# r-mafi/ClaraGenomicsAnalysis

Hardware: AMD Instinct MI355X
Metric: POA windows/sec (consensus) (higher is better)
Workload: dtype int16

## Files before the change

### claragenomicsanalysis_amd/csrc/poa_common.hpp

```cpp
#pragma once

#include <cstddef>
#include <cstdint>

namespace gwamd
{
namespace poa
{

constexpr int kMaxEdges      = 50;
constexpr int kMaxAlignments = 50;
constexpr int kBandPad       = 8;
constexpr int kWave          = 64;
constexpr int kCellsPerLane  = 8;
constexpr int kChunk         = kWave * kCellsPerLane;
constexpr int kAdRing        = 128;
constexpr int kAdSpillDist   = kAdRing - kWave + 1;
constexpr int band_ring_rows(int cpl) { return cpl >= 16 ? 8 : 16; }
constexpr int band_tile_rows(int cpl) { return cpl >= 10 ? 32 : 64; }
constexpr int kReadGuard     = 64;
constexpr int kAdMaxWaves    = 4;
constexpr int kColShift      = 7;

enum Status : uint8_t
{
    kSuccess               = 0,
    kExceededMaxPoas       = 1,
    kExceededMaxSeqSize    = 2,
    kExceededMaxSeqsPerPoa = 3,
    kNodeCountExceeded     = 4,
    kEdgeCountExceeded     = 5,
    kSeqLenExceededNodes   = 6,
    kLoopCountExceeded     = 7,
    kOutputTypeUnavailable = 8,
    kGenericError          = 9,
};

struct WindowDesc
{
    int32_t first_seq;
    int32_t num_seqs;
};

struct Dims
{
    int32_t max_nodes;
    int32_t max_seqs;
    int32_t max_seq_len;
    int32_t max_consensus;
    int32_t score_stride;
    int32_t score_rows;
    int32_t aln_cap;
    int32_t band_width;
    int32_t want_consensus;
    int32_t spoa_accurate;
    int32_t lds_kernel;
    int32_t lds_bytes;
    int32_t lds_ring_off;
    int32_t lds_ring_rows;
    int32_t lds_sh_off;
    int32_t lds_rec_off;
    int32_t lds_xl_off;
    int32_t lds_xl_cap;
    int32_t lds_cpl;
    int32_t lds_waves;
    int32_t code_stride;
    int64_t aux_stride;
    int32_t aux_carry_off;
    int32_t lds_work_bytes;
    int32_t aux_reca_off;
    int32_t aux_recb_off;
    int32_t aux_col0_off;
    int32_t aux_flag_off;
    int32_t aux_xl_off;
    int32_t aux_xl_cap;
    int32_t aux_bx_off;
    int32_t aux_recc_off;
    int32_t aux_rece_off;
    int32_t band_ad;
    int32_t tb_rank;
    int32_t diag;
};

constexpr int kTbRanked     = 1;
constexpr int kTbStrips     = 2;
constexpr int kTbStrip32    = 4;
constexpr int kTbDefault    = kTbRanked | kTbStrips;
constexpr int kTbAboveShift = 3;
constexpr int kTbAboveMask  = 7;

constexpr int kDiagTopsortRing  = 1;
constexpr int kDiagFwdV1        = 2;
constexpr int kDiagTopsortFifo  = 4;
constexpr int kDiagRaconV1      = 8;
constexpr int kDiagConsensusHbm = 16;
constexpr int kDiagAddWave0     = 32;
constexpr int kDiagAddSerial    = 64;
constexpr int kDiagOrderKahn    = 128;
constexpr int kDiagSinkCap2     = 256;
constexpr int kDiagConsLdsShift = 16;

struct LdsShape
{
    int cpl, waves;
    bool wide;
};
constexpr LdsShape kLdsShapes[] = {{8, 1, true},   {8, 2, true},   {8, 4, true},   {8, 8, true},  {16, 8, true},
                                   {8, 1, false},  {16, 1, false}, {24, 1, false}, {32, 1, false}, {8, 2, false},
                                   {8, 3, false},  {8, 4, false},  {16, 4, false}, {4, 4, false}};
constexpr int kNumLdsShapes = int(sizeof(kLdsShapes) / sizeof(kLdsShapes[0]));

struct KernelRef
{
    const void* fn;
    int threads;
    size_t dynamic_lds;
};

constexpr int64_t lds_read_bytes(int64_t max_seq_len) { return (max_seq_len + 48 + 15) & ~int64_t(15); }

constexpr int kAddShBytes = 64;
constexpr int64_t lds_add_ms(int64_t max_seq_len) { return (max_seq_len + 16) & ~int64_t(15); }
constexpr int64_t lds_add_wave0_bytes(int64_t max_seq_len, int64_t max_nodes)
{
    return 5 * lds_add_ms(max_seq_len) + 2 * (max_nodes + max_seq_len);
}
constexpr int64_t lds_add_hit_off(int64_t max_seq_len, int64_t max_nodes)
{
    return (lds_add_wave0_bytes(max_seq_len, max_nodes) + 15) & ~int64_t(15);
}
constexpr int64_t lds_add_bytes(int64_t max_seq_len, int64_t max_nodes)
{
    return lds_add_hit_off(max_seq_len, max_nodes) + 2 * lds_add_ms(max_seq_len) + kAddShBytes;
}
constexpr bool lds_add_fits(int64_t max_seq_len, int64_t max_nodes, int64_t ring_bytes)
{
    return max_seq_len > 0 && max_nodes > 0 && max_nodes + max_seq_len < 65535 &&
           lds_add_bytes(max_seq_len, max_nodes) <= ring_bytes;
}

constexpr int kTbRankBytes = 7 * 144 + 128 * 4;

constexpr int kShProg    = 16;
constexpr int kShEnd     = 32;
constexpr int kShBnd     = 64;
constexpr int kShChan    = 128;
constexpr int kChanRows  = 64;
constexpr int kMaxWaves  = 4;
constexpr int kShBytes(int waves) { return kShChan + (waves - 1) * kChanRows * 4; }
constexpr int kShEndW   = 32;
constexpr int kShProgW  = 64;
constexpr int kShBndW   = 128;
constexpr int kShChanW  = 384;
constexpr int kMaxRingW = 8;
constexpr int kShBytesW(int waves) { return kShChanW + (waves - 1) * kChanRows * 8; }

constexpr int kTileRows = 128;
constexpr int kTileCols = 128;
constexpr int kTileXlMin = 512;

struct Buffers
{
    const uint8_t* seqs;
    const int8_t* wts;
    const int32_t* seq_len;
    const int64_t* seq_off;
    const WindowDesc* windows;
    const int32_t* order;
    int32_t num_windows;
    int32_t* head;
    int32_t num_slots;
    uint8_t* base;
    uint16_t* in_cnt;
    uint16_t* out_cnt;
    uint16_t* aln_cnt;
    uint16_t* node_cov;
    uint16_t* in_w;
    void* in_e;
    void* out_e;
    void* aln;
    void* sorted;
    void* pos;
    void* ag;
    void* ar;
    void* scores;
    uint8_t* codes;
    int32_t* cscore;
    void* cpred;
    uint16_t* edge_cov;
    uint16_t* edge_cov_cnt;
    void* seq_begin;
    uint8_t* cons;
    uint16_t* cov;
    int32_t* cons_len;
    uint8_t* status;
    uint8_t* msa_status;
    uint8_t* msa;
    int32_t* msa_len;
    int32_t* final_nodes;
    int64_t* cells;
    int64_t* phase;
    int32_t* order_stats;
};

enum OrderStat
{
    kOsSpliced = 0,
    kOsSortSeqAdd,
    kOsSortCheck,
    kOsSortNoOld,
    kOsSortSinkCap,
    kOsSortEmptyRead,
    kOsSortLast,
    kOsTieSorts,
    kOsTieQuick,
    kOsSortAfterTie,
    kOrderStats
};


enum Phase
{
    kPhBackbone = 0,
    kPhForward,
    kPhTraceback,
    kPhAdd,
    kPhTopsort,
    kPhOutput,
// ... 13 lines not shown
```

### claragenomicsanalysis_amd/csrc/poa_fwd2.hpp

```cpp
#pragma once

__device__ __forceinline__ bool fwd2_ok(const Scores sc)
{
    const int s_eq = sc.match - sc.gap, s_ne = sc.mismatch - sc.gap;
    return s_eq >= 0 && s_eq <= 255 && s_ne >= 0 && s_ne <= 255;
}

__device__ __forceinline__ int wave_incl_max_b(int v)
{
    v = max(v, __builtin_amdgcn_update_dpp(INT_MIN, v, 0x111, 0xf, 0xf, false));
    v = max(v, __builtin_amdgcn_update_dpp(INT_MIN, v, 0x112, 0xf, 0xf, false));
    v = max(v, __builtin_amdgcn_update_dpp(INT_MIN, v, 0x114, 0xf, 0xf, false));
    v = max(v, __builtin_amdgcn_update_dpp(INT_MIN, v, 0x118, 0xf, 0xf, false));
    v = max(v, __builtin_amdgcn_update_dpp(INT_MIN, v, 0x142, 0xa, 0xf, false));
    v = max(v, __builtin_amdgcn_update_dpp(INT_MIN, v, 0x143, 0xc, 0xf, false));
    return v;
}

typedef u32x4 fwd_u32x4;
typedef u32x2 fwd_u32x2;

template <int NR>
__device__ __forceinline__ void load_row_glb(const GWAMD_GLB int16_t* p, uint32_t (&P)[NR], uint32_t& prev)
{
    static_assert(NR % 4 == 0 || NR == 2, "4 or a multiple of 8 cells per lane");
    if constexpr (NR % 4 == 0)
    {
#pragma unroll
        for (int q = 0; q < NR / 4; q++)
        {
            const fwd_u32x4 v = *reinterpret_cast<const GWAMD_GLB fwd_u32x4*>(p + 1 + 8 * q);
            P[4 * q] = v.x, P[4 * q + 1] = v.y, P[4 * q + 2] = v.z, P[4 * q + 3] = v.w;
        }
    }
    else
    {
        const fwd_u32x2 v = *reinterpret_cast<const GWAMD_GLB fwd_u32x2*>(p + 1);
        P[0] = v.x, P[1] = v.y;
    }
    prev = uint32_t(uint16_t(p[0]));
}

template <int NR>
__device__ __forceinline__ void load_row_lds(const GWAMD_LDS int16_t* p, uint32_t (&P)[NR], uint32_t& prev)
{
    static_assert(NR % 4 == 0 || NR == 2, "4 or a multiple of 8 cells per lane");
    if constexpr (NR % 4 == 0)
    {
#pragma unroll
        for (int q = 0; q < NR / 4; q++)
        {
            const fwd_u32x4 v = *reinterpret_cast<const GWAMD_LDS fwd_u32x4*>(p + 1 + 8 * q);
            P[4 * q] = v.x, P[4 * q + 1] = v.y, P[4 * q + 2] = v.z, P[4 * q + 3] = v.w;
        }
    }
    else
    {
        const fwd_u32x2 v = *reinterpret_cast<const GWAMD_LDS fwd_u32x2*>(p + 1);
        P[0] = v.x, P[1] = v.y;
    }
    prev = uint32_t(uint16_t(p[0]));
}

template <int CPL, int NW, bool FIRST, bool FEED, typename SizeT>
__device__ __forceinline__ void fwd2_rows(WinGraph<SizeT> g, const RowProg& P, int V, const uint8_t* read_f, int L,
                                          int16_t* ring_f, int ring_stride, int16_t* spill_f, int stride,
                                          uint8_t* codes_f, int code_stride, const Scores sc,
                                          GWAMD_LDS uint8_t* shb, int16_t* carry_f, int lane, int wave, int cb,
                                          bool to_hbm, bool from_hbm, bool owner, int xl_cap, int& best_row,
                                          int& best_val)
{
    g = as_global(g);
    GWAMD_LDS int16_t* ring          = lds_of(ring_f);
    const GWAMD_LDS uint8_t* read    = lds_of(read_f);
    const GWAMD_LDS uint32_t* prec   = lds_of(P.rec);
    const GWAMD_LDS uint16_t* pxl    = lds_of(P.xl);
    GWAMD_GLB int16_t* spill         = (GWAMD_GLB int16_t*)(spill_f);
    GWAMD_GLB uint8_t* codes         = (GWAMD_GLB uint8_t*)(codes_f);
    GWAMD_GLB int16_t* carry_hbm     = (GWAMD_GLB int16_t*)(carry_f);
    constexpr int NR    = CPL / 2;
    const int gap       = sc.gap;
    const int s_eq      = sc.match - gap;
    const int s_ne      = sc.mismatch - gap;
    const uint32_t gap2 = pk_bcast(gap);
    const uint32_t one2 = opaque_u32(0x00010001u);
    const uint32_t two2 = opaque_u32(0x00020002u);
    const int mask      = uniform(P.ring_mask);
    GWAMD_LDS int16_t* bnd               = (GWAMD_LDS int16_t*)(shb + kShBnd) + wave * (mask + 1);
    GWAMD_LDS uint32_t* chan             = (GWAMD_LDS uint32_t*)(shb + kShChan);
    volatile GWAMD_LDS uint32_t* chan_in  = chan + (wave - 1) * kChanRows;
    volatile GWAMD_LDS uint32_t* chan_out = chan + wave * kChanRows;
    volatile GWAMD_LDS int* prog_v        = (GWAMD_LDS int*)(shb + kShProg);
    const int jb     = cb + lane * CPL;
    const bool active = jb < L;
    const int ja     = active ? jb : 0;
    const int own_lane = ((L > 0 ? L - 1 : 0) % (kWave * CPL)) / CPL;
    const int own_c    = (L > 0 ? L - 1 : 0) % CPL;
    const int xl_last = xl_cap;

    uint32_t T[CPL];
#pragma unroll
    for (int c = 0; c < CPL; c++)
    {
        const int ch = int(read[ja + c]);
        T[c] = uint32_t(ch == 'A' ? s_eq : s_ne) | (uint32_t(ch == 'C' ? s_eq : s_ne) << 8) |
               (uint32_t(ch == 'T' ? s_eq : s_ne) << 16) | (uint32_t(ch == 'G' ? s_eq : s_ne) << 24);
    }
    uint32_t Eprev[NR];
#pragma unroll
    for (int i = 0; i < NR; i++)
        Eprev[i] = 0;
    int cin_prev = 0;
    int hbm_c    = 0;
    uint32_t rec_c = uint32_t(uniform(int(prec[1])));
    uint32_t rec_n = uint32_t(uniform(int(prec[min(2, V)])));
    auto xls_at = [&](int i) { return int(pxl[i]); };
    int pv_c = xls_at(min(int(rec_c >> 16), xl_last) + lane);
    GWAMD_GLB uint8_t* crow = codes + code_stride;
    GWAMD_GLB int16_t* srow = spill + stride;
    for (int r = 1; r <= V; r++, crow += code_stride, srow += stride)
    {
        const uint32_t rec = rec_c;
        const uint32_t rec_nn = prec[min(r + 2, V)];
        const int pv_n = xls_at(min(int(rec_n >> 16), xl_last) + lane);
        const int np       = int((rec >> 8) & 63);
        const bool spill_r = (rec >> 15) & 1;
        GWAMD_LDS int16_t* row = ring + (r & mask) * ring_stride;
        uint32_t sig[NR];
        {
            const uint32_t bsel = 0x0c040c00u + ((rec >> 1) & 3u) * 0x00010001u;
#pragma unroll
            for (int i = 0; i < NR; i++)
                sig[i] = __builtin_amdgcn_perm(T[2 * i + 1], T[2 * i], bsel);
        }
        int cin = 0;
        auto finish = [&](auto multi_tag, const uint32_t(&dg)[NR], const uint32_t(&vt)[NR],
                          const uint32_t(&kd)[NR], const uint32_t(&kv)[NR], int c0v,
                          int c0kv) __attribute__((always_inline)) {
            constexpr bool kMulti = decltype(multi_tag)::value;
            uint32_t E[NR];
#pragma unroll
            for (int i = 0; i < NR; i++)
            {
                const uint32_t s = pk_max_lo_into_hi(pk_max(dg[i], vt[i]));
                E[i]             = i == 0 ? s : pk_max_hi_carry(s, E[i - 1]);
            }
            const int m    = active ? int(int16_t(E[NR - 1] >> 16)) : kNeg;
            const int incl = wave_incl_max_b(m);
            const int excl = __builtin_amdgcn_update_dpp(kNeg, incl, 0x138, 0xf, 0xf, false);
            const int wtot = __builtin_amdgcn_readlane(incl, kWave - 1);
            if (FIRST)
            {
                cin = c0v + gap;
                if (lane == 0)
                {
                    row[kColShift]  = int16_t(cin);
                    crow[kColShift] = uint8_t(1 | (c0kv << 2));
                    if (spill_r)
                        srow[kColShift] = int16_t(cin);
                }
            }
            else
            {
                if (from_hbm)
                {
                    if (((r - 1) & (kWave - 1)) == 0)
                    {
                        const int x = r + lane;
                        uint32_t hc = x <= V ? uint32_t(int(carry_hbm[x])) : 0u;
                        settle_vm1(hc);
                        hbm_c = int(hc);
                    }
                    cin = int(int16_t(__builtin_amdgcn_readlane(hbm_c, (r - 1) & (kWave - 1))));
                }
                else
                {
                    uint32_t w = uint32_t(uniform(int(chan_in[r & (kChanRows - 1)])));
                    while ((w >> 16) != (uint32_t(r) & 0xffffu))
                    {
                        __builtin_amdgcn_s_sleep(1);
                        w = uint32_t(uniform(int(chan_in[r & (kChanRows - 1)])));
                    }
                    cin = int(int16_t(w & 0xffffu));
                    if ((r & 7) == 0 && lane == 0)
                        prog_v[wave] = r;
                }
                if (lane == 0)
                {
                    bnd[r & mask] = int16_t(cin);
                    if (spill_r)
                        srow[cb + kColShift] = int16_t(cin);
                }
            }
            if (FEED)
            {
                if ((r & 31) == 0 && r >= kChanRows)
                {
                    while (uniform(prog_v[wave + 1]) < r - 32)
                        __builtin_amdgcn_s_sleep(1);
                }
                if (lane == 0)
                    chan_out[r & (kChanRows - 1)] = (uint32_t(r) << 16) | uint32_t(uint16_t(max(cin, wtot)));
            }
            if (to_hbm && lane == 0)
                carry_hbm[r] = int16_t(max(cin, wtot));
            const uint32_t b2v = pk_bcast(max(excl, cin));
#pragma unroll
            for (int i = 0; i < NR; i++)
                E[i] = pk_max(E[i], b2v);
            if (active)
            {
                uint32_t code[NR];
#pragma unroll
                for (int i = 0; i < NR; i++)
                {
                    if constexpr (kMulti)
                    {
                        const uint32_t a   = pk_min_u(pk_sub(E[i], dg[i]), one2);
                        const uint32_t bb  = pk_min_u(pk_sub(E[i], vt[i]), one2);
                        const uint32_t cvh = pk_mad(bb, pk_sub(two2, kv[i]), kv[i]);
                        code[i]            = pk_mad(a, pk_sub(cvh, kd[i]), kd[i]);
                    }
                    else
                    {
                        const uint32_t a = pk_min_u(pk_sub(E[i], dg[i]), one2);
                        code[i]          = pk_add(a, pk_min_u(pk_sub(E[i], vt[i]), a));
                    }
                }
                if constexpr (NR % 4 == 0)
                {
#pragma unroll
                    for (int q = 0; q < NR / 4; q++)
                    {
                        const fwd_u32x4 ev = {E[4 * q], E[4 * q + 1], E[4 * q + 2], E[4 * q + 3]};
                        *reinterpret_cast<GWAMD_LDS fwd_u32x4*>(row + jb + kColShift + 1 + 8 * q) = ev;
                        if (spill_r)
                            *reinterpret_cast<GWAMD_GLB fwd_u32x4*>(srow + jb + kColShift + 1 + 8 * q) = ev;
                        const uint32_t w0 = __builtin_amdgcn_perm(code[4 * q + 1], code[4 * q], 0x06040200u);
                        const uint32_t w1 = __builtin_amdgcn_perm(code[4 * q + 3], code[4 * q + 2], 0x06040200u);
                        __builtin_nontemporal_store(uint64_t(w0) | (uint64_t(w1) << 32),
                                                    reinterpret_cast<GWAMD_GLB uint64_t*>(crow + jb + kColShift + 1 + 8 * q));
                    }
                }
                else
                {
                    const fwd_u32x2 ev = {E[0], E[1]};
                    *reinterpret_cast<GWAMD_LDS fwd_u32x2*>(row + jb + kColShift + 1) = ev;
                    if (spill_r)
                        *reinterpret_cast<GWAMD_GLB fwd_u32x2*>(srow + jb + kColShift + 1) = ev;
                    __builtin_nontemporal_store(__builtin_amdgcn_perm(code[1], code[0], 0x06040200u),
                                                reinterpret_cast<GWAMD_GLB uint32_t*>(crow + jb + kColShift + 1));
                }
            }
            if ((rec & (1u << 14)) && owner)
            {
                int endv = cin;
#pragma unroll
                for (int i = 0; i < NR; i++)
                {
                    if (2 * i == own_c)
                        endv = int(int16_t(E[i] & 0xffff));
                    if (2 * i + 1 == own_c)
                        endv = int(int16_t(E[i] >> 16));
                }
                const int v = L == 0 ? cin : __builtin_amdgcn_readlane(endv, own_lane);
                if (best_val < v)
                    best_val = v, best_row = r;
            }
#pragma unroll
            for (int i = 0; i < NR; i++)
                Eprev[i] = E[i];
        };
        if (!(rec & 0x80u) && np == 1)
        {
            const int d = int(rec >> 16);
            uint32_t prev;
            if (d == 1)
                prev = uint32_t(__builtin_amdgcn_update_dpp(int(uint32_t(uint16_t(cin_prev))),
                                                            int(Eprev[NR - 1] >> 16), 0x138, 0xf, 0xf, false));
            else
            {
                const int ps = (r - d) & mask;
                load_row_lds<NR>(ring + ps * ring_stride + ja + kColShift, Eprev, prev);
                if (!FIRST)
                {
                    const uint32_t bv = uint32_t(uint16_t(bnd[ps]));
                    prev              = lane == 0 ? bv : prev;
                }
            }
            const int c0v = FIRST ? int(int16_t(__builtin_amdgcn_readfirstlane(prev))) : 0;
            uint32_t dg[NR], vt[NR];
            diag_src<NR>(Eprev, prev, dg);
#pragma unroll
            for (int i = 0; i < NR; i++)
            {
                dg[i] = pk_add(dg[i], sig[i]);
                vt[i] = pk_add(Eprev[i], gap2);
            }
            finish(std::false_type{}, dg, vt, dg, vt, c0v, 0);
        }
        else
        {
            auto rows_general = [&](auto slow_tag, int pv, int n) __attribute__((always_inline)) {
                constexpr bool kSlow = decltype(slow_tag)::value;
                auto load_pred = [&](int p, uint32_t(&Q)[NR], uint32_t& qprev) __attribute__((always_inline)) {
                    if (p == r - 1)
                    {
#pragma unroll
                        for (int i = 0; i < NR; i++)
                            Q[i] = Eprev[i];
                        qprev = uint32_t(__builtin_amdgcn_update_dpp(int(uint32_t(uint16_t(cin_prev))),
                                                                     int(Eprev[NR - 1] >> 16), 0x138, 0xf, 0xf,
                                                                     false));
                        return;
                    }
                    if constexpr (kSlow)
                    {
                        if (p == 0)
                        {
#pragma unroll
                            for (int i = 0; i < NR; i++)
                                Q[i] = 0;
                            qprev = 0;
                            return;
                        }
                        if (r - p > mask)
                        {
                            load_row_glb<NR>(spill + size_t(p) * stride + ja + kColShift, Q, qprev);
                            settle_vm<NR>(Q, qprev);
                            return;
                        }
                    }
                    load_row_lds<NR>(ring + (p & mask) * ring_stride + ja + kColShift, Q, qprev);
                    if (!FIRST)
                    {
                        const uint32_t bv = uint32_t(uint16_t(bnd[p & mask]));
                        qprev             = lane == 0 ? bv : qprev;
                    }
                };
                uint32_t dg[NR], vt[NR];
                int c0v = 0, c0kv = 0;
                {
                    uint32_t Pv[NR], prev;
                    load_pred(__builtin_amdgcn_readfirstlane(pv), Pv, prev);
                    if (FIRST)
                        c0v = int(int16_t(__builtin_amdgcn_readfirstlane(prev)));
                    diag_src<NR>(Pv, prev, dg);
#pragma unroll
                    for (int i = 0; i < NR; i++)
                    {
                        dg[i] = pk_add(dg[i], sig[i]);
                        vt[i] = pk_add(Pv[i], gap2);
                    }
                }
                if (n > 1)
                {
                    uint32_t kd[NR], kv[NR];
#pragma unroll
                    for (int i = 0; i < NR; i++)
                    {
                        kd[i] = 0;
                        kv[i] = one2;
                    }
                    for (int k = 1; k < n; k++)
                    {
                        uint32_t Q[NR], qprev, dq[NR];
                        load_pred(__builtin_amdgcn_readlane(pv, k), Q, qprev);
                        if (FIRST)
                        {
                            const int pe = int(int16_t(__builtin_amdgcn_readfirstlane(qprev)));
                            c0kv         = pe > c0v ? k : c0kv;
                            c0v          = max(c0v, pe);
                        }
                        diag_src<NR>(Q, qprev, dq);
                        const uint32_t kk4 = pk_bcast(4 * k);
                        const uint32_t kk1 = pk_bcast(4 * k + 1);
#pragma unroll
                        for (int i = 0; i < NR; i++)
                        {
                            const uint32_t d  = pk_add(dq[i], sig[i]);
                            const uint32_t nd = pk_max(dg[i], d);
                            kd[i] = pk_mad(pk_min_u(pk_sub(nd, dg[i]), one2), pk_sub(kk4, kd[i]), kd[i]);
                            dg[i] = nd;
                            const uint32_t v  = pk_add(Q[i], gap2);
                            const uint32_t nv = pk_max(vt[i], v);
                            kv[i] = pk_mad(pk_min_u(pk_sub(nv, vt[i]), one2), pk_sub(kk1, kv[i]), kv[i]);
                            vt[i] = nv;
                        }
                    }
                    finish(std::true_type{}, dg, vt, kd, kv, c0v, c0kv);
                }
                else
                    finish(std::false_type{}, dg, vt, dg, vt, c0v, 0);
            };
            if (!(rec & 0x80u))
                rows_general(std::false_type{}, pv_c, np);
            else
            {
                int n  = np;
                int pv = 0;
                if (np == int(kRecEscape))
                    pv = row_preds<SizeT>(P, g, r, rec, lane, n);
                else
                {
                    if (np >= 2)
                        pv = lane < np ? int(pxl[(rec >> 16) + lane]) : 0;
                    else if (np == 1)
                        pv = r - int(rec >> 16);
                    if (np == 0)
                        n = 1;
                }
                const uint32_t ub = uint32_t(row_base<SizeT>(g, rec, r));
                if (!((ub & 0xc0u) == 0x40u && ((0x10008aull >> (ub & 0x3fu)) & 1u)))
                {
                    const GWAMD_LDS uint32_t* rw = reinterpret_cast<const GWAMD_LDS uint32_t*>(read + ja);
#pragma unroll
                    for (int i = 0; i < NR; i++)
                    {
                        const uint32_t wv = rw[i / 2] >> ((i & 1) * 16);
                        const int ch0 = int(wv & 0xff), ch1 = int((wv >> 8) & 0xff);
                        sig[i]        = uint32_t(uint16_t(ch0 == int(ub) ? s_eq : s_ne)) |
                                 (uint32_t(uint16_t(ch1 == int(ub) ? s_eq : s_ne)) << 16);
                    }
                }
                rows_general(std::true_type{}, pv, uniform(n));
            }
        }
        cin_prev = cin;
        rec_c    = rec_n;
        rec_n    = uint32_t(uniform(int(rec_nn)));
        pv_c     = pv_n;
    }
}

template <int CPL, int NW, typename SizeT>
__device__ int nw_forward_lds_v2(WinGraph<SizeT> g, const RowProg& P, int V, const uint8_t* read, int L,
                                 int16_t* ring, int ring_stride, int16_t* spill, int stride, uint8_t* codes,
                                 int code_stride, const Scores sc, GWAMD_LDS uint8_t* shb, int16_t* carry_hbm,
                                 int tid, int xl_cap)
{
    constexpr int kSpan = kWave * CPL;
    const int lane      = tid & (kWave - 1);
    const int wave      = uniform(tid / kWave);
    V                   = uniform(V);
    L                   = uniform(L);
    const int jl        = L > 0 ? L - 1 : 0;
    const int own_span  = jl / kSpan;
    const int nspan     = max(1, (L + kSpan - 1) / kSpan);
    const int nsweep    = (nspan + NW - 1) / NW;
    int best_row        = 0;
    int best_val        = INT_MIN;
    for (int sweep = 0; sweep < nsweep; sweep++)
    {
        if (sweep > 0)
        {
            __syncthreads();
            for (int t = tid; t < (kShChan - kShProg) / 4 + (NW - 1) * kChanRows; t += kWave * NW)
                reinterpret_cast<GWAMD_LDS int*>(shb + kShProg)[t] = 0;
            __syncthreads();
        }
        const int span      = sweep * NW + wave;
        const int cb        = span * kSpan;
        const bool first    = span == 0;
        const bool wact     = cb < L || first;
        const bool feed     = wave + 1 < NW && cb + kSpan < L;
        const bool to_hbm   = wave == NW - 1 && cb + kSpan < L;
        const bool from_hbm = wave == 0 && sweep > 0;
        const bool owner    = span == own_span;
        if (!wact || V < 1)
            continue;
        if (first)
        {
            if (feed)
                fwd2_rows<CPL, NW, true, true>(g, P, V, read, L, ring, ring_stride, spill, stride, codes,
                                               code_stride, sc, shb, carry_hbm, lane, wave, cb, to_hbm, from_hbm,
                                               owner, xl_cap, best_row, best_val);
            else
                fwd2_rows<CPL, NW, true, false>(g, P, V, read, L, ring, ring_stride, spill, stride, codes,
                                                code_stride, sc, shb, carry_hbm, lane, wave, cb, to_hbm,
                                                from_hbm, owner, xl_cap, best_row, best_val);
        }
        else if (feed)
            fwd2_rows<CPL, NW, false, true>(g, P, V, read, L, ring, ring_stride, spill, stride, codes, code_stride,
                                            sc, shb, carry_hbm, lane, wave, cb, to_hbm, from_hbm, owner, xl_cap,
                                            best_row, best_val);
        else
            fwd2_rows<CPL, NW, false, false>(g, P, V, read, L, ring, ring_stride, spill, stride, codes,
                                             code_stride, sc, shb, carry_hbm, lane, wave, cb, to_hbm, from_hbm,
                                             owner, xl_cap, best_row, best_val);
    }
    if (nsweep > 1 || NW > 1)
    {
        GWAMD_LDS int* endp = (GWAMD_LDS int*)(shb + kShEnd);
        if (wave == own_span % NW && lane == 0)
            *endp = best_row;
        __syncthreads();
        best_row = uniform(*endp);
    }
    return best_row;
}
```

### claragenomicsanalysis_amd/csrc/poa_kernels.hip

```cpp
#include <hip/hip_runtime.h>

#include <climits>
#include <cstdint>
#include <type_traits>
#include <utility>

#include "poa_wave.hpp"
#include "poa_order.hpp"
#include "poa_rowprog.hpp"

namespace gwamd
{
namespace poa
{

template <typename ScoreT, typename SizeT, bool BANDED, bool MSA>
__global__ void __launch_bounds__(kWave) poa_window_kernel(Buffers b, Dims d, Scores sc)
{
    extern __shared__ __align__(16) uint8_t lds_read[];
    __shared__ int sh_alen;
    __shared__ int sh_status;
    __shared__ int sh_len;

    const int w = b.order ? b.order[blockIdx.x] : int(blockIdx.x);
// ... 154 lines not shown
    return __builtin_bit_cast(uint32_t, __builtin_elementwise_min(__builtin_bit_cast(pk_u16x2, a),
                                                                  __builtin_bit_cast(pk_u16x2, b)));
}
__device__ __forceinline__ uint32_t pk_mad(uint32_t a, uint32_t b, uint32_t c)
{
    return __builtin_bit_cast(uint32_t, __builtin_bit_cast(pk_u16x2, a) * __builtin_bit_cast(pk_u16x2, b) +
                                            __builtin_bit_cast(pk_u16x2, c));
}
__device__ __forceinline__ uint32_t opaque_u32(uint32_t v)
{
    asm volatile("" : "+v"(v));
    return v;
}
__device__ __forceinline__ uint32_t pk_bcast(int v) { return (uint32_t(uint16_t(v)) * 0x10001u); }
__device__ __forceinline__ uint32_t pk_max_lo_into_hi(uint32_t a)
{
    const pk_s16x2 v = __builtin_bit_cast(pk_s16x2, a);
    return __builtin_bit_cast(uint32_t, __builtin_elementwise_max(v, __builtin_shufflevector(v, v, 0, 0)));
}
__device__ __forceinline__ uint32_t pk_max_hi_carry(uint32_t a, uint32_t c)
{
    const pk_s16x2 v = __builtin_bit_cast(pk_s16x2, c);
    return __builtin_bit_cast(uint32_t, __builtin_elementwise_max(__builtin_bit_cast(pk_s16x2, a),
                                                                  __builtin_shufflevector(v, v, 1, 1)));
}

__device__ __forceinline__ void settle_vm1(uint32_t& v) { asm volatile("" : "+v"(v)); }
template <int NR>
__device__ __forceinline__ void settle_vm(uint32_t (&P)[NR], uint32_t& prev)
{
#pragma unroll
    for (int i = 0; i < NR; i++)
        settle_vm1(P[i]);
    settle_vm1(prev);
}

template <int NR>
__device__ __forceinline__ void load_pred_pk(const int16_t* ring, int ring_stride, int ring_mask, const int16_t* spill,
                                             int stride, int r, int p, int jb, uint32_t (&P)[NR], uint32_t& prev)
{
    const int16_t* lrow = ring + (p & ring_mask) * ring_stride + jb + kColShift;
#pragma unroll
    for (int q = 0; q < NR / 4; q++)
    {
        const uint4 v = *reinterpret_cast<const uint4*>(lrow + 1 + 8 * q);
        P[4 * q] = v.x, P[4 * q + 1] = v.y, P[4 * q + 2] = v.z, P[4 * q + 3] = v.w;
    }
    prev = uint32_t(uint16_t(lrow[0]));
    if (p == 0)
    {
#pragma unroll
        for (int i = 0; i < NR; i++)
            P[i] = 0;
        prev = 0;
    }
    else if (r - p > ring_mask)
    {
        const int16_t* grow = spill + size_t(p) * stride + jb + kColShift;
#pragma unroll
        for (int q = 0; q < NR / 4; q++)
        {
            const uint4 v = *reinterpret_cast<const uint4*>(grow + 1 + 8 * q);
            P[4 * q] = v.x, P[4 * q + 1] = v.y, P[4 * q + 2] = v.z, P[4 * q + 3] = v.w;
        }
        prev = uint32_t(uint16_t(grow[0]));
        settle_vm<NR>(P, prev);
    }
}

template <int NR>
__device__ __forceinline__ void diag_src(const uint32_t (&P)[NR], uint32_t prev, uint32_t (&Dg)[NR])
{
    Dg[0] = __builtin_amdgcn_alignbyte(P[0], prev << 16, 2);
#pragma unroll
    for (int i = 1; i < NR; i++)
        Dg[i] = __builtin_amdgcn_alignbyte(P[i], P[i - 1], 2);
}

#ifdef GWAMD_FWD_PROFILE
struct FwdProf
{
    uint64_t t[8] = {0, 0, 0, 0, 0, 0, 0, 0};
    uint64_t m    = 0;
    __device__ void start() { m = __builtin_amdgcn_s_memtime(); }
    template <int I>
    __device__ void lap()
    {
        const uint64_t x = __builtin_amdgcn_s_memtime();
        t[I] += x - m;
        m = x;
    }
};
#define GWAMD_FP_START(fp) fp.start()
#define GWAMD_FP_LAP(fp, I) fp.template lap<I>()
#else
struct FwdProf
{
};
#define GWAMD_FP_START(fp)
#define GWAMD_FP_LAP(fp, I)
#endif

template <typename SizeT>
__device__ __forceinline__ int row_preds(const RowProg& P, WinGraph<SizeT> g, int rr, uint32_t rec, int lane,
                                         int& n)
{
    g = as_global(g);
    n      = int((rec >> 8) & 63);
    int pv = 0;
    if (n == int(kRecEscape))
    {
        const int node = uniform(int(g.sorted[rr - 1]));
        n              = uniform(int(g.in_cnt[node]));
        uint32_t t     = lane < n ? uint32_t(pred_row(g, node, lane)) : 0u;
        settle_vm1(t);
        pv = int(t);
    }
    else if (n >= 2)
        pv = lane < n ? int(P.xl[(rec >> 16) + lane]) : 0;
    else if (n == 1)
        pv = rr - int(rec >> 16);
    if (n == 0)
        n = 1;
    return pv;
}

template <int NR>
__device__ __forceinline__ void load_row_pk(const int16_t* p, uint32_t (&P)[NR], uint32_t& prev)
{
    if constexpr (NR % 4 == 0)
    {
#pragma unroll
        for (int q = 0; q < NR / 4; q++)
        {
            const uint4 v = *reinterpret_cast<const uint4*>(p + 1 + 8 * q);
            P[4 * q] = v.x, P[4 * q + 1] = v.y, P[4 * q + 2] = v.z, P[4 * q + 3] = v.w;
        }
    }
    else
    {
        static_assert(NR == 2, "4 or a multiple of 8 cells per lane");
        const uint2 v = *reinterpret_cast<const uint2*>(p + 1);
        P[0] = v.x, P[1] = v.y;
    }
    prev = uint32_t(uint16_t(p[0]));
}

template <int CPL, int NW, typename SizeT>
__device__ int nw_forward_lds_pk(WinGraph<SizeT> g, const RowProg& P, int V, const uint8_t* read, int L,
                                 int16_t* ring, int ring_stride, int16_t* spill, int stride, uint8_t* codes,
                                 int code_stride, const Scores sc, GWAMD_LDS uint8_t* shb, int16_t* carry_hbm,
                                 int tid, FwdProf& fp)
{
    g = as_global(g);
    constexpr int NR    = CPL / 2;
    constexpr int kSpan = kWave * CPL;
    const int lane      = tid & (kWave - 1);
    const int wave      = uniform(tid / kWave);
    V                   = uniform(V);
    L                   = uniform(L);
    const int gap       = sc.gap;
    const int s_eq      = sc.match - gap;
    const int s_ne      = sc.mismatch - gap;
    const uint32_t gap2 = pk_bcast(gap);
    const uint32_t one2 = opaque_u32(0x00010001u);
    const uint32_t two2 = opaque_u32(0x00020002u);
    const int mask      = uniform(P.ring_mask);
    GWAMD_LDS int* prog          = (GWAMD_LDS int*)(shb + kShProg);
    GWAMD_LDS int16_t* bnd       = (GWAMD_LDS int16_t*)(shb + kShBnd) + wave * (mask + 1);
    GWAMD_LDS uint32_t* chan     = (GWAMD_LDS uint32_t*)(shb + kShChan);
    volatile GWAMD_LDS uint32_t* chan_in  = chan + (wave - 1) * kChanRows;
    volatile GWAMD_LDS uint32_t* chan_out = chan + wave * kChanRows;
    volatile GWAMD_LDS int* prog_v        = prog;
    const int jl        = L > 0 ? L - 1 : 0;
    const int own_span  = jl / kSpan;
    const int own_lane  = (jl % kSpan) / CPL;
    const int own_c     = jl % CPL;
    const int nspan     = max(1, (L + kSpan - 1) / kSpan);
    const int nsweep    = (nspan + NW - 1) / NW;
    int best_row        = 0;
    int best_val        = INT_MIN;
    for (int sweep = 0; sweep < nsweep; sweep++)
    {
// ... 524 lines not shown
            eg = i == pi ? -1 : i;
            er = j == pj ? -1 : j - 1;
        }
        n++;
        if ((n & (kWave - 1)) == 0)
            flush(n);
        i = pi;
        j = pj;
    }
    if ((n & (kWave - 1)) != 0)
        flush(n);
    wave_sync();
    if (loops >= bound || n > aln_cap)
        return -1;
    return n;
}

#include "poa_fwd2.hpp"
#include "poa_fwd_w.hpp"

template <bool MSA, int CPL, int NW, bool W>
__global__ void __launch_bounds__(kWave * NW, W ? (NW >= 8 ? 2 : 1) : (NW >= 4 ? 2 : 1))
    poa_window_kernel_lds(Buffers b, Dims d, Scores sc)
{
    using SizeT  = int16_t;
    using RowT   = typename std::conditional<W, int32_t, int16_t>::type;
    extern __shared__ __align__(16) uint8_t lds[];
    __shared__ int sh_status;
    __shared__ int sh_len;

    __shared__ int sh_next;
    if (int(blockIdx.x) >= b.num_windows)
        return;
    const int tid      = threadIdx.x;
    const int lane     = tid & (kWave - 1);
    const int wave     = uniform(tid / kWave);
    constexpr int kThr = kWave * NW;
    const size_t slot  = blockIdx.x;

    uint8_t* lread   = lds;
    RowT* ring       = reinterpret_cast<RowT*>(lds + d.lds_ring_off);
    uint8_t* tile    = lds + d.lds_ring_off;
    const int rstride = d.score_stride;
    GWAMD_LDS uint8_t* shb = (GWAMD_LDS uint8_t*)(lds) + d.lds_sh_off;
    const AddScratch AX = lds_add_scratch((GWAMD_LDS uint8_t*)(lds) + d.lds_ring_off, d.max_seq_len, d.max_nodes,
                                          false, (GWAMD_LDS int*)(shb));
    const bool add_fits = lds_add_fits(d.max_seq_len, d.max_nodes, d.lds_rec_off - d.lds_ring_off);
    const int add_mode  = (d.diag & kDiagAddSerial) ? 2 : (((d.diag & kDiagAddWave0) || !add_fits) ? 1 : 0);

    for (int idx = blockIdx.x; idx < b.num_windows;)
    {
    const int w     = b.order ? b.order[idx] : idx;
    const size_t mn = size_t(d.max_nodes);
    WinGraph<SizeT> g;
    g.base      = b.base + w * mn;
    g.in_cnt    = b.in_cnt + w * mn;
    g.out_cnt   = b.out_cnt + w * mn;
    g.aln_cnt   = b.aln_cnt + w * mn;
    g.cov       = b.node_cov + w * mn;
    g.in_w      = b.in_w + w * mn * kMaxEdges;
    g.in_e      = static_cast<SizeT*>(b.in_e) + w * mn * kMaxEdges;
    g.out_e     = static_cast<SizeT*>(b.out_e) + w * mn * kMaxEdges;
    g.aln       = static_cast<SizeT*>(b.aln) + w * mn * kMaxAlignments;
    g.sorted    = static_cast<SizeT*>(b.sorted) + w * mn;
    g.pos       = static_cast<SizeT*>(b.pos) + w * mn;
    g.max_nodes = d.max_nodes;

    SizeT* ag        = static_cast<SizeT*>(b.ag) + slot * d.aln_cap;
    SizeT* ar        = static_cast<SizeT*>(b.ar) + slot * d.aln_cap;
    RowT* spill      = static_cast<RowT*>(b.scores) + slot * d.score_rows * size_t(rstride);
    uint8_t* codes   = b.codes + slot * size_t(d.aux_stride);
    uint32_t* rec    = reinterpret_cast<uint32_t*>(lds + d.lds_rec_off);
    uint16_t* xl     = reinterpret_cast<uint16_t*>(lds + d.lds_xl_off);
    RowT* carry      = reinterpret_cast<RowT*>(codes + d.aux_carry_off);
    RowProg P{rec, xl, d.lds_ring_rows - 1};
    int32_t* cscore  = b.cscore + slot * mn;
    SizeT* cpred     = static_cast<SizeT*>(b.cpred) + slot * mn * 4;
    uint16_t* ecov   = MSA ? b.edge_cov + w * mn * kMaxEdges * d.max_seqs : nullptr;
    uint16_t* ecovc  = MSA ? b.edge_cov_cnt + w * mn * kMaxEdges : nullptr;
    SizeT* seq_begin = MSA ? static_cast<SizeT*>(b.seq_begin) + size_t(w) * d.max_seqs : nullptr;

    PhaseTimer ph;
    FwdProf fp;
#ifdef GWAMD_FWD_PROFILE
    const bool use_v2 = false;
#else
    const bool use_v2 = !W && fwd2_ok(sc) && !(d.diag & kDiagFwdV1);
#endif
    const WindowDesc wd = b.windows[w];
    const int nseq      = wd.num_seqs;
    int status          = kSuccess;
    int64_t cells       = 0;
    int node_count      = 0;
    int lv_hint         = 0;
    bool order_kahn = true;
    bool splice_on  = !d.spoa_accurate && !(d.diag & (kDiagTopsortFifo | kDiagOrderKahn));
    int tie_hold    = 0;
    const int sink_cap = (d.diag & kDiagSinkCap2) ? 2 : kSinkCap;
    const int xcap  = d.lds_xl_cap - kSinkWords;
    GWAMD_LDS uint16_t* sinks = (GWAMD_LDS uint16_t*)(lds + d.lds_xl_off) + xcap;
    int32_t* ostat  = b.order_stats + size_t(w) * kOrderStats;
    auto count      = [&](int k) {
        if (tid == 0)
            __hip_atomic_fetch_add(ostat + k, 1, __ATOMIC_RELAXED, __HIP_MEMORY_SCOPE_AGENT);
    };
    if (tid < kOrderStats)
        ostat[tid] = 0;
    auto kahn_sort = [&](WinGraph<SizeT> gx, int n, int n_prev) {
        const bool done = topsort_levels<SizeT, NW>(gx, n, n_prev, (GWAMD_LDS uint8_t*)(lds), d.lds_sh_off, tid,
                                                    kThr, cpred, lv_hint);
        if (!done && tid == 0)
            topsort_kahn<SizeT>(gx, n, cscore);
        lv_hint = done ? n : 0;
        __syncthreads();
    };

    if (nseq > 0)
    {
        const int len0      = b.seq_len[wd.first_seq];
        const uint8_t* seq0 = b.seqs + b.seq_off[wd.first_seq];
        const int8_t* w0    = b.wts + b.seq_off[wd.first_seq];
        if (wave == 0)
            build_backbone<SizeT, MSA>(g, seq0, w0, len0, lane, ecov, ecovc, seq_begin, d.max_seqs);
        node_count = len0;
        ph.lap<kPhBackbone>();
        for (int s = 1; s < nseq; s++)
        {
            if (node_count >= d.max_nodes)
            {
                status = kNodeCountExceeded;
                break;
            }
            const int L           = b.seq_len[wd.first_seq + s];
            const int64_t off     = b.seq_off[wd.first_seq + s];
            const uint8_t* read_g = b.seqs + off;
            const int8_t* wts_g   = b.wts + off;
            const int padded      = (L + 32 + 15) & ~15;
            const int V           = node_count;
            auto stage_and_program = [&]() {
                for (int j = tid; j < padded; j += kThr)
                    lread[j] = j < L ? read_g[j] : 0;
                build_row_program<NW, NW + (W ? 16 : 0)>(lds_kernel_args(), w, V, (GWAMD_LDS uint8_t*)(lds));
            };
            auto stage_and_program_w0 = [&]() {
                for (int j = tid; j < padded; j += kThr)
                    lread[j] = j < L ? read_g[j] : 0;
                if (wave == 0)
                    build_row_program_wave0<SizeT>(g, V, rec, xl, xcap, d.lds_ring_rows, lane,
                                                   (GWAMD_LDS uint8_t*)(lds) + d.lds_ring_off, sinks);
            };
            stage_and_program();
            if (NW > 1)
            {
                constexpr int kP = W ? kShProgW : kShProg;
                constexpr int kB = W ? kShBytesW(NW) : kShBytes(NW);
                for (int t = tid; t < (kB - kP) / 4; t += kThr)
                    reinterpret_cast<GWAMD_LDS int*>(shb + kP)[t] = 0;
            }
            __syncthreads();
            int nsink = (order_kahn && tie_hold == 0) ? 1 : uniform(int(sinks[kSinkCap]));
            if (nsink > sink_cap && order_kahn)
                nsink = 1;
            if (nsink > sink_cap)
            {
                __syncthreads();
                kahn_sort(g, V, V);
                count(kOsSortSinkCap);
                order_kahn = true;
                splice_on  = false;
                nsink      = 1;
                stage_and_program_w0();
                __syncthreads();
            }
            ph.lap<kPhRowProg>();
            cells += int64_t(V + 1) * (L + 1);
            int end_row;
            if constexpr (W)
                end_row = nw_forward_lds_w<CPL, NW, SizeT>(g, P, V, lread, L, ring, rstride, spill, rstride, codes,
                                                           d.code_stride, sc, shb, carry, tid);
            else if constexpr (CPL <= 16)
                end_row = use_v2 ? nw_forward_lds_v2<CPL, NW, SizeT>(g, P, V, lread, L, ring, rstride, spill, rstride,
                                                                     codes, d.code_stride, sc, shb, carry, tid,
                                                                     d.lds_xl_cap)
                                 : nw_forward_lds_pk<CPL, NW, SizeT>(g, P, V, lread, L, ring, rstride, spill, rstride,
                                                                     codes, d.code_stride, sc, shb, carry, tid, fp);
            else
                end_row = nw_forward_lds_pk<CPL, NW, SizeT>(g, P, V, lread, L, ring, rstride, spill, rstride, codes,
                                                            d.code_stride, sc, shb, carry, tid, fp);
            __syncthreads();
            ph.lap<kPhForward>();
            if (nsink >= 2)
            {
                int srow_l = 0, sval = INT_MIN, smax = INT_MIN;
                bool tied  = false;
                if (wave == 0)
                {
                    if (lane < nsink)
                    {
                        srow_l = int(sinks[lane]);
                        sval   = int(glb(spill)[size_t(srow_l) * rstride + L + kColShift]);
                    }
                    smax              = wave_max(sval);
                    tied              = lane < nsink && sval == smax;
                    const uint64_t tm = __builtin_amdgcn_ballot_w64(tied);
                    int code = 0, er = end_row;
                    if (__popcll(tm) >= 2)
                    {
                        int node = 0, ic = 0, pr = -1;
                        if (tied)
                        {
                            node = int(glb(g.sorted)[srow_l - 1]);
                            ic   = int(glb(g.in_cnt)[node]);
                            pr   = ic == 1 ? int(glb(g.in_e)[node * kMaxEdges]) : -1;
                        }
                        const int p0 = __builtin_amdgcn_readlane(pr, uniform(__builtin_ctzll(tm)));
                        if (__builtin_amdgcn_ballot_w64(tied && (ic != 1 || pr != p0)) == 0)
                        {
                            int slot = INT_MAX;
                            if (tied)
                            {
                                const int oc = int(glb(g.out_cnt)[p0]);
                                for (int e = oc - 1; e >= 0; e--)
                                    if (int(glb(g.out_e)[p0 * kMaxEdges + e]) == node)
                                        slot = e;
                            }
                            const int smin = -wave_max(-slot);
                            const uint64_t m = __builtin_amdgcn_ballot_w64(tied && slot == smin);
                            er   = __builtin_amdgcn_readlane(srow_l, uniform(__builtin_ctzll(m)));
                            code = 1;
                        }
                        else
                            code = 2;
                    }
                    if (lane == 0)
                        sh_len = code | (er << 2);
                }
                __syncthreads();
                const int tv = uniform(sh_len);
                __syncthreads();
                const int code = tv & 3;
                if (code == 1 && !order_kahn)
                {
                    end_row = tv >> 2;
                    count(kOsTieQuick);
                }
                if (code == 2 && !order_kahn)
                {
                    WinGraph<SizeT> gk = g;
                    gk.sorted          = cpred + mn;
                    gk.pos             = cpred + 2 * mn;
                    for (int i = tid; i < V; i += kThr)
                        glb(gk.sorted)[i] = glb(g.sorted)[i];
                    kahn_sort(gk, V, V);
                    count(kOsTieSorts);
                    if (wave == 0)
                    {
                        int kp = INT_MAX;
                        if (tied)
                            kp = int(glb(gk.pos)[int(glb(g.sorted)[srow_l - 1])]);
                        const int kmin = -wave_max(-kp);
                        const uint64_t m = __builtin_amdgcn_ballot_w64(kp == kmin);
                        const int er   = __builtin_amdgcn_readlane(srow_l, uniform(__builtin_ctzll(m)));
                        if (lane == 0)
                            sh_len = er;
                    }
                    __syncthreads();
// ... 268 lines not shown
```

Baseline: 18840.

## Hand over inter-wave boundary carries in blocks through a lane register

Replaces the per-row LDS channel handshake between waves in the v2 forward pass with block handover: each producer wave collects 16 boundary values in a register (one per lane slot), publishes them to LDS once per block, and bumps a head counter. The consumer waits once per block, loads the whole block into a lane-indexed register, and reads the boundary with readlane instead of the per-row bnd ring in LDS. This cuts per-row polling and LDS traffic between pipelined waves. The cost is coarser-grained dependency, which adds pipeline latency between waves. The change also adds profiling hooks that compile away by default.

```diff
diff --git a/claragenomicsanalysis_amd/csrc/poa_common.hpp b/claragenomicsanalysis_amd/csrc/poa_common.hpp
--- a/claragenomicsanalysis_amd/csrc/poa_common.hpp
+++ b/claragenomicsanalysis_amd/csrc/poa_common.hpp
@@ -2,6 +2,8 @@
 
 #include <cstddef>
 #include <cstdint>
+
+#include "poa_handover.hpp"
 
 namespace gwamd
 {
@@ -143,7 +145,9 @@
 
 constexpr int kShProg    = 16;
 constexpr int kShEnd     = 32;
+constexpr int kShHead    = 48;
 constexpr int kShBnd     = 64;
+constexpr int kMaxRingRows16 = 8;
 constexpr int kShChan    = 128;
 constexpr int kChanRows  = 64;
 constexpr int kMaxWaves  = 4;
diff --git a/claragenomicsanalysis_amd/csrc/poa_fwd2.hpp b/claragenomicsanalysis_amd/csrc/poa_fwd2.hpp
--- a/claragenomicsanalysis_amd/csrc/poa_fwd2.hpp
+++ b/claragenomicsanalysis_amd/csrc/poa_fwd2.hpp
@@ -1,4 +1,11 @@
 #pragma once
+
+#ifndef GWAMD_HAND_BLOCK
+#define GWAMD_HAND_BLOCK 16
+#endif
+constexpr int kHandBlock = GWAMD_HAND_BLOCK;
+
+__device__ __forceinline__ int write_lane(int v, int x, int sel, int lane) { return lane == sel ? x : v; }
 
 __device__ __forceinline__ bool fwd2_ok(const Scores sc)
 {
@@ -62,14 +69,16 @@
     prev = uint32_t(uint16_t(p[0]));
 }
 
-template <int CPL, int NW, bool FIRST, bool FEED, typename SizeT>
+template <int CPL, int NW, bool FIRST, bool FEED, int HB, typename SizeT>
 __device__ __forceinline__ void fwd2_rows(WinGraph<SizeT> g, const RowProg& P, int V, const uint8_t* read_f, int L,
                                           int16_t* ring_f, int ring_stride, int16_t* spill_f, int stride,
                                           uint8_t* codes_f, int code_stride, const Scores sc,
                                           GWAMD_LDS uint8_t* shb, int16_t* carry_f, int lane, int wave, int cb,
                                           bool to_hbm, bool from_hbm, bool owner, int xl_cap, int& best_row,
-                                          int& best_val)
+                                          int& best_val, FwdProf& fp)
 {
+    static_assert(HB == 0 || (hand_block_ok(HB) && HB + kMaxRingRows16 <= kHandSlots && kChanRows == kHandSlots),
+                  "a block and the ring's reach fit the 64 lanes of the carry register");
     g = as_global(g);
     GWAMD_LDS int16_t* ring          = lds_of(ring_f);
     const GWAMD_LDS uint8_t* read    = lds_of(read_f);
@@ -91,6 +100,7 @@
     volatile GWAMD_LDS uint32_t* chan_in  = chan + (wave - 1) * kChanRows;
     volatile GWAMD_LDS uint32_t* chan_out = chan + wave * kChanRows;
     volatile GWAMD_LDS int* prog_v        = (GWAMD_LDS int*)(shb + kShProg);
+    volatile GWAMD_LDS int* head_v        = (GWAMD_LDS int*)(shb + kShHead);
     const int jb     = cb + lane * CPL;
     const bool active = jb < L;
     const int ja     = active ? jb : 0;
@@ -111,15 +121,55 @@
     for (int i = 0; i < NR; i++)
         Eprev[i] = 0;
     int cin_prev = 0;
-    int hbm_c    = 0;
+    int cv  = 0;
+    int pvr = 0;
     uint32_t rec_c = uint32_t(uniform(int(prec[1])));
     uint32_t rec_n = uint32_t(uniform(int(prec[min(2, V)])));
     auto xls_at = [&](int i) { return int(pxl[i]); };
     int pv_c = xls_at(min(int(rec_c >> 16), xl_last) + lane);
     GWAMD_GLB uint8_t* crow = codes + code_stride;
     GWAMD_GLB int16_t* srow = spill + stride;
+    GWAMD_FP_START(fp);
     for (int r = 1; r <= V; r++, crow += code_stride, srow += stride)
     {
+        if constexpr (HB > 0)
+        {
+            GWAMD_FP_MARK(fp, 4);
+            if (!FIRST && hand_opens(r, HB))
+            {
+                if (from_hbm)
+                {
+                    const int x = hand_lane_row(lane, r);
+                    uint32_t hc = x >= 1 && x <= V ? uint32_t(int(carry_hbm[x])) : 0u;
+                    settle_vm1(hc);
+                    cv = hand_lane_in_block(lane, r, HB) ? int(hc) : cv;
+                }
+                else
+                {
+                    const int need = hand_need_head(r, V, HB);
+                    while (uniform(head_v[wave - 1]) < need)
+                    {
+                        GWAMD_FP_COUNT(fp, 4);
+                        __builtin_amdgcn_s_sleep(1);
+                    }
+                    const int w = int(chan_in[lane]);
+                    cv          = hand_lane_in_block(lane, r, HB) ? w : cv;
+                    if (lane == 0)
+                        prog_v[wave] = hand_new_tail(r, V, HB);
+                }
+            }
+            if (FEED && hand_opens(r, HB) && hand_must_wait(r))
+            {
+                const int need = hand_free_tail(r, HB);
+                while (uniform(prog_v[wave + 1]) < need)
+                {
+                    GWAMD_FP_COUNT(fp, 5);
+                    __builtin_amdgcn_s_sleep(1);
+                }
+            }
+            GWAMD_FP_LAP(fp, 4);
+        }
+        GWAMD_FP_COUNT(fp, 7);
         const uint32_t rec = rec_c;
         const uint32_t rec_nn = prec[min(r + 2, V)];
         const int pv_n = xls_at(min(int(rec_n >> 16), xl_last) + lane);
@@ -133,6 +183,7 @@
             for (int i = 0; i < NR; i++)
                 sig[i] = __builtin_amdgcn_perm(T[2 * i + 1], T[2 * i], bsel);
         }
+        GWAMD_FP_LAP(fp, 0);
         int cin = 0;
         auto finish = [&](auto multi_tag, const uint32_t(&dg)[NR], const uint32_t(&vt)[NR],
                           const uint32_t(&kd)[NR], const uint32_t(&kv)[NR], int c0v,
@@ -149,6 +200,8 @@
             const int incl = wave_incl_max_b(m);
             const int excl = __builtin_amdgcn_update_dpp(kNeg, incl, 0x138, 0xf, 0xf, false);
             const int wtot = __builtin_amdgcn_readlane(incl, kWave - 1);
+            GWAMD_FP_LAP(fp, 3);
+            GWAMD_FP_MARK(fp, 4);
             if (FIRST)
             {
                 cin = c0v + gap;
@@ -162,22 +215,25 @@
             }
             else
             {
-                if (from_hbm)
+                if constexpr (HB > 0)
+                    cin = int(int16_t(__builtin_amdgcn_readlane(cv, hand_slot(r))));
+                else if (from_hbm)
                 {
                     if (((r - 1) & (kWave - 1)) == 0)
                     {
                         const int x = r + lane;
                         uint32_t hc = x <= V ? uint32_t(int(carry_hbm[x])) : 0u;
                         settle_vm1(hc);
-                        hbm_c = int(hc);
-                    }
-                    cin = int(int16_t(__builtin_amdgcn_readlane(hbm_c, (r - 1) & (kWave - 1))));
+                        cv = int(hc);
+                    }
+                    cin = int(int16_t(__builtin_amdgcn_readlane(cv, (r - 1) & (kWave - 1))));
                 }
                 else
                 {
                     uint32_t w = uint32_t(uniform(int(chan_in[r & (kChanRows - 1)])));
                     while ((w >> 16) != (uint32_t(r) & 0xffffu))
                     {
+                        GWAMD_FP_COUNT(fp, 4);
                         __builtin_amdgcn_s_sleep(1);
                         w = uint32_t(uniform(int(chan_in[r & (kChanRows - 1)])));
                     }
@@ -187,23 +243,33 @@
                 }
                 if (lane == 0)
                 {
-                    bnd[r & mask] = int16_t(cin);
+                    if constexpr (HB == 0)
+                        bnd[r & mask] = int16_t(cin);
                     if (spill_r)
                         srow[cb + kColShift] = int16_t(cin);
                 }
             }
             if (FEED)
             {
-                if ((r & 31) == 0 && r >= kChanRows)
-                {
-                    while (uniform(prog_v[wave + 1]) < r - 32)
-                        __builtin_amdgcn_s_sleep(1);
-                }
-                if (lane == 0)
-                    chan_out[r & (kChanRows - 1)] = (uint32_t(r) << 16) | uint32_t(uint16_t(max(cin, wtot)));
+                if constexpr (HB > 0)
+                    pvr = write_lane(pvr, max(cin, wtot), hand_slot(r), lane);
+                else
+                {
+                    if ((r & 31) == 0 && r >= kChanRows)
+                    {
+                        while (uniform(prog_v[wave + 1]) < r - 32)
+                        {
+                            GWAMD_FP_COUNT(fp, 5);
+                            __builtin_amdgcn_s_sleep(1);
+                        }
+                    }
+                    if (lane == 0)
+                        chan_out[r & (kChanRows - 1)] = (uint32_t(r) << 16) | uint32_t(uint16_t(max(cin, wtot)));
+                }
             }
             if (to_hbm && lane == 0)
                 carry_hbm[r] = int16_t(max(cin, wtot));
+            GWAMD_FP_LAP(fp, 4);
             const uint32_t b2v = pk_bcast(max(excl, cin));
 #pragma unroll
             for (int i = 0; i < NR; i++)
@@ -252,6 +318,7 @@
                                                 reinterpret_cast<GWAMD_GLB uint32_t*>(crow + jb + kColShift + 1));
                 }
             }
+            GWAMD_FP_LAP(fp, 5);
             if ((rec & (1u << 14)) && owner)
             {
                 int endv = cin;
@@ -276,15 +343,20 @@
             const int d = int(rec >> 16);
             uint32_t prev;
             if (d == 1)
+            {
+                GWAMD_FP_COUNT(fp, 0);
                 prev = uint32_t(__builtin_amdgcn_update_dpp(int(uint32_t(uint16_t(cin_prev))),
                                                             int(Eprev[NR - 1] >> 16), 0x138, 0xf, 0xf, false));
+            }
             else
             {
+                GWAMD_FP_COUNT(fp, 1);
                 const int ps = (r - d) & mask;
                 load_row_lds<NR>(ring + ps * ring_stride + ja + kColShift, Eprev, prev);
                 if (!FIRST)
                 {
-                    const uint32_t bv = uint32_t(uint16_t(bnd[ps]));
+                    const uint32_t bv = HB > 0 ? uint32_t(__builtin_amdgcn_readlane(cv, hand_slot(r - d))) & 0xffffu
+                                               : uint32_t(uint16_t(bnd[ps]));
                     prev              = lane == 0 ? bv : prev;
                 }
             }
@@ -297,6 +369,7 @@
                 dg[i] = pk_add(dg[i], sig[i]);
                 vt[i] = pk_add(Eprev[i], gap2);
             }
+            GWAMD_FP_LAP(fp, 1);
             finish(std::false_type{}, dg, vt, dg, vt, c0v, 0);
         }
         else
@@ -334,7 +407,8 @@
                     load_row_lds<NR>(ring + (p & mask) * ring_stride + ja + kColShift, Q, qprev);
                     if (!FIRST)
                     {
-                        const uint32_t bv = uint32_t(uint16_t(bnd[p & mask]));
+                        const uint32_t bv = HB > 0 ? uint32_t(__builtin_amdgcn_readlane(cv, hand_slot(p))) & 0xffffu
+                                                   : uint32_t(uint16_t(bnd[p & mask]));
                         qprev             = lane == 0 ? bv : qprev;
                     }
                 };
@@ -388,15 +462,23 @@
                             vt[i] = nv;
                         }
                     }
+                    GWAMD_FP_LAP(fp, 2);
                     finish(std::true_type{}, dg, vt, kd, kv, c0v, c0kv);
                 }
                 else
+                {
+                    GWAMD_FP_LAP(fp, 2);
                     finish(std::false_type{}, dg, vt, dg, vt, c0v, 0);
+                }
             };
             if (!(rec & 0x80u))
+            {
+                GWAMD_FP_COUNT(fp, 2);
                 rows_general(std::false_type{}, pv_c, np);
+            }
             else
             {
+                GWAMD_FP_COUNT(fp, 3);
                 int n  = np;
                 int pv = 0;
                 if (np == int(kRecEscape))
@@ -426,18 +508,32 @@
                 rows_general(std::true_type{}, pv, uniform(n));
             }
         }
+        if constexpr (HB > 0)
+        {
+            if (FEED && hand_closes(r, V, HB))
+            {
+                GWAMD_FP_MARK(fp, 4);
+                if (hand_lane_in_block(lane, r, HB))
+                    chan_out[lane] = uint32_t(pvr);
+                if (lane == 0)
+                    head_v[wave] = r;
+                GWAMD_FP_LAP(fp, 4);
+            }
+        }
         cin_prev = cin;
         rec_c    = rec_n;
         rec_n    = uint32_t(uniform(int(rec_nn)));
         pv_c     = pv_n;
-    }
+        GWAMD_FP_LAP(fp, 6);
+    }
+    GWAMD_FP_STOP(fp);
 }
 
 template <int CPL, int NW, typename SizeT>
 __device__ int nw_forward_lds_v2(WinGraph<SizeT> g, const RowProg& P, int V, const uint8_t* read, int L,
                                  int16_t* ring, int ring_stride, int16_t* spill, int stride, uint8_t* codes,
                                  int code_stride, const Scores sc, GWAMD_LDS uint8_t* shb, int16_t* carry_hbm,
-                                 int tid, int xl_cap)
+                                 int tid, int xl_cap, FwdProf& fp)
 {
     constexpr int kSpan = kWave * CPL;
     const int lane      = tid & (kWave - 1);
@@ -469,25 +565,22 @@
         const bool owner    = span == own_span;
         if (!wact || V < 1)
             continue;
+        auto rows = [&](auto first_tag, auto feed_tag) __attribute__((always_inline)) {
+            fwd2_rows<CPL, NW, decltype(first_tag)::value, decltype(feed_tag)::value, kHandBlock>(
+                g, P, V, read, L, ring, ring_stride, spill, stride, codes, code_stride, sc, shb, carry_hbm, lane, wave,
+                cb, to_hbm, from_hbm, owner, xl_cap, best_row, best_val, fp);
+        };
         if (first)
         {
             if (feed)
-                fwd2_rows<CPL, NW, true, true>(g, P, V, read, L, ring, ring_stride, spill, stride, codes,
-                                               code_stride, sc, shb, carry_hbm, lane, wave, cb, to_hbm, from_hbm,
-                                               owner, xl_cap, best_row, best_val);
+                rows(std::true_type{}, std::true_type{});
             else
-                fwd2_rows<CPL, NW, true, false>(g, P, V, read, L, ring, ring_stride, spill, stride, codes,
-                                                code_stride, sc, shb, carry_hbm, lane, wave, cb, to_hbm,
-                                                from_hbm, owner, xl_cap, best_row, best_val);
+                rows(std::true_type{}, std::false_type{});
         }
         else if (feed)
-            fwd2_rows<CPL, NW, false, true>(g, P, V, read, L, ring, ring_stride, spill, stride, codes, code_stride,
-                                            sc, shb, carry_hbm, lane, wave, cb, to_hbm, from_hbm, owner, xl_cap,
-                                            best_row, best_val);
+            rows(std::false_type{}, std::true_type{});
         else
-            fwd2_rows<CPL, NW, false, false>(g, P, V, read, L, ring, ring_stride, spill, stride, codes,
-                                             code_stride, sc, shb, carry_hbm, lane, wave, cb, to_hbm, from_hbm,
-                                             owner, xl_cap, best_row, best_val);
+            rows(std::false_type{}, std::false_type{});
     }
     if (nsweep > 1 || NW > 1)
     {
diff --git a/claragenomicsanalysis_amd/csrc/poa_handover.hpp b/claragenomicsanalysis_amd/csrc/poa_handover.hpp
--- /dev/null
+++ b/claragenomicsanalysis_amd/csrc/poa_handover.hpp
@@ -0,0 +1,27 @@
+#pragma once
+
+namespace gwamd
+{
+namespace poa
+{
+
+constexpr int kHandSlots = 64;
+
+constexpr bool hand_block_ok(int B) { return B >= 1 && B <= kHandSlots && kHandSlots % B == 0; }
+
+constexpr int hand_slot(int r) { return r & (kHandSlots - 1); }
+constexpr int hand_block_slot(int r, int B) { return hand_slot(r) & ~(B - 1); }
+constexpr bool hand_lane_in_block(int lane, int r, int B) { return (lane & ~(B - 1)) == hand_block_slot(r, B); }
+constexpr int hand_lane_row(int lane, int r) { return (r & ~(kHandSlots - 1)) + lane; }
+
+constexpr bool hand_opens(int r, int B) { return (r & (B - 1)) == 0 || r == 1; }
+constexpr bool hand_closes(int r, int V, int B) { return (r & (B - 1)) == B - 1 || r == V; }
+constexpr int hand_block_last(int r, int V, int B) { return (r | (B - 1)) < V ? (r | (B - 1)) : V; }
+
+constexpr int hand_need_head(int r, int V, int B) { return hand_block_last(r, V, B); }
+constexpr int hand_new_tail(int r, int V, int B) { return hand_block_last(r, V, B); }
+constexpr bool hand_must_wait(int r) { return r >= kHandSlots; }
+constexpr int hand_free_tail(int r, int B) { return (r | (B - 1)) - kHandSlots; }
+
+}
+}
diff --git a/claragenomicsanalysis_amd/csrc/poa_kernels.hip b/claragenomicsanalysis_amd/csrc/poa_kernels.hip
--- a/claragenomicsanalysis_amd/csrc/poa_kernels.hip
+++ b/claragenomicsanalysis_amd/csrc/poa_kernels.hip
@@ -260,6 +260,38 @@
 {
     uint64_t t[8] = {0, 0, 0, 0, 0, 0, 0, 0};
     uint64_t m    = 0;
+#ifdef GWAMD_FWD_PROFILE_COUNTS
+    __device__ void start() {}
+    template <int I>
+    __device__ void lap()
+    {
+    }
+    template <int I>
+    __device__ void count()
+    {
+        t[I] += 1;
+    }
+#elif defined(GWAMD_FWD_PROFILE_ONLY)
+    uint64_t m0 = 0;
+    __device__ void start() { m0 = __builtin_amdgcn_s_memtime(); }
+    __device__ void stop() { t[7] += __builtin_amdgcn_s_memtime() - m0; }
+    template <int I>
+    __device__ void mark()
+    {
+        if (I == GWAMD_FWD_PROFILE_ONLY)
+            m = __builtin_amdgcn_s_memtime();
+    }
+    template <int I>
+    __device__ void lap()
+    {
+        if (I == GWAMD_FWD_PROFILE_ONLY)
+            t[I] += __builtin_amdgcn_s_memtime() - m;
+    }
+    template <int I>
+    __device__ void count()
+    {
+    }
+#else
     __device__ void start() { m = __builtin_amdgcn_s_memtime(); }
     template <int I>
     __device__ void lap()
@@ -268,15 +300,33 @@
         t[I] += x - m;
         m = x;
     }
+    template <int I>
+    __device__ void count()
+    {
+    }
+#endif
+#ifndef GWAMD_FWD_PROFILE_ONLY
+    __device__ void stop() {}
+    template <int I>
+    __device__ void mark()
+    {
+    }
+#endif
 };
 #define GWAMD_FP_START(fp) fp.start()
+#define GWAMD_FP_STOP(fp) fp.stop()
+#define GWAMD_FP_MARK(fp, I) fp.template mark<I>()
 #define GWAMD_FP_LAP(fp, I) fp.template lap<I>()
+#define GWAMD_FP_COUNT(fp, I) fp.template count<I>()
 #else
 struct FwdProf
 {
 };
 #define GWAMD_FP_START(fp)
+#define GWAMD_FP_STOP(fp)
+#define GWAMD_FP_MARK(fp, I)
 #define GWAMD_FP_LAP(fp, I)
+#define GWAMD_FP_COUNT(fp, I)
 #endif
 
 template <typename SizeT>
@@ -967,11 +1017,7 @@
 
     PhaseTimer ph;
     FwdProf fp;
-#ifdef GWAMD_FWD_PROFILE
-    const bool use_v2 = false;
-#else
     const bool use_v2 = !W && fwd2_ok(sc) && !(d.diag & kDiagFwdV1);
-#endif
     const WindowDesc wd = b.windows[w];
     const int nseq      = wd.num_seqs;
     int status          = kSuccess;
@@ -1066,7 +1112,7 @@
             else if constexpr (CPL <= 16)
                 end_row = use_v2 ? nw_forward_lds_v2<CPL, NW, SizeT>(g, P, V, lread, L, ring, rstride, spill, rstride,
                                                                      codes, d.code_stride, sc, shb, carry, tid,
-                                                                     d.lds_xl_cap)
+                                                                     d.lds_xl_cap, fp)
                                  : nw_forward_lds_pk<CPL, NW, SizeT>(g, P, V, lread, L, ring, rstride, spill, rstride,
                                                                      codes, d.code_stride, sc, shb, carry, tid, fp);
             else
```

Result: faster. 19300 (median of 6 runs) (+2.4%).
